# Sanoojan/VFace

Hardware: AMD Instinct MI355X
Metric: swapped frames/sec at 512x512, 50-step DDIM (higher is better)
Workload: dtype f16

## Files before the change

### include/vface_hip.h

```cpp
#ifndef VFACE_HIP_H
#define VFACE_HIP_H

#include <stddef.h>
#include <stdint.h>

#ifdef __cplusplus
extern "C" {
#endif

#define VFACE_ABI_VERSION 8

#define VFACE_OK 0
#define VFACE_ERR_ARG (-1)
#define VFACE_ERR_ALIGN (-2)
#define VFACE_ERR_SHAPE (-3)
#define VFACE_ERR_DTYPE (-4)
#define VFACE_ERR_LAUNCH (-5)
#define VFACE_ERR_WORKSPACE (-6)

#define VFACE_F16 0
#define VFACE_BF16 1

#define VFACE_EPI_GEGLU 1
#define VFACE_EPI_OUT_F32 2
#define VFACE_TUNE_VARIANT(v) ((v) << 8)
#define VFACE_CONV_PAD_TRAILING 0x40000
#define VFACE_TUNE_NO_PERSISTENT 0x10000
#define VFACE_TUNE_PERSISTENT 0x20000
#define VFACE_TUNE_NO_PATCH 0x80000
#define VFACE_TUNE_PATCH 0x100000
#define VFACE_TUNE_GN8 0x8000000
#define VFACE_TUNE_NO_Q8 0x4000000
#define VFACE_TUNE_PATCH_BN160 0x2000000
#define VFACE_TUNE_F32_TRANSPOSE 0x1000000
#define VFACE_TUNE_BIG_TILE 0x10000000
#define VFACE_TUNE_NO_BIG_TILE 0x20000000
#define VFACE_TUNE_BIG_W256 0x200000
#define VFACE_TUNE_BIG_W320 0x400000

#define VFACE_FUSION_NONE 0
#define VFACE_FUSION_REPLACE 1
#define VFACE_FUSION_LINEAR 2

int vface_abi_version(void);
const char* vface_error_string(int code);
int vface_gemm_variants_built(void);

typedef struct vface_stream32 {
    const float* residual32;
    int64_t ldr32;
    float* out32;
    int64_t ldo32;
    const float* in_scale_shift;
// ... 191 lines not shown
```

### vface_amd/csrc/conv.hip

```cpp
#include <type_traits>
#include "common.hpp"
#include "vface_kernels.hpp"

namespace {

constexpr int TP = 16;

template <class TT, int NT, int KH, int KW, bool DIAG = false, bool GNT = false, int RM = -1, bool Q8 = false>
__global__ __launch_bounds__(512, 2) void conv_patch_kernel(GemmParams p) {
    using E = typename TT::elem;
    using V8 = typename TT::v8;
    constexpr int BN = 32 * NT;
    constexpr int TAPS = KH * KW;
    static_assert(!Q8 || (KH == 3 && KW == 3 && NT == 4), "the 8x8 form: 3x3 windows, 128-channel tiles");
    constexpr int PW = Q8 ? 20 : TP + KW - 1, PH = Q8 ? 20 : TP + KH - 1, NPIX = PW * PH;
    constexpr int NPIECES = (NPIX + 7) / 8;
    constexpr int PATCH_BYTES = NPIECES * 1024;
    constexpr int PPW = (NPIECES + 7) / 8;
    constexpr int BPIECES = BN / 8;
    constexpr int BSLOT = BN * 128;
    constexpr int NB_HI = (BPIECES + 7) / 8, NB_LO = BPIECES / 8;
    constexpr int NB_SPLIT = BPIECES % 8;
    constexpr int NSLOT = (TAPS % 3 == 0) ? 3 : 4;
    static_assert(TAPS % NSLOT == 0 && (NSLOT - 1) * BSLOT < 65536, "slot offsets must fold into the ds_read immediate");
    extern __shared__ __attribute__((aligned(16))) unsigned char smem_raw[];
    unsigned char* sB = smem_raw;
    unsigned char* sP = smem_raw + NSLOT * BSLOT;
    constexpr bool GNF = GNT && KH == 3;
    unsigned char* sT = sP + 2 * PATCH_BYTES;
// ... 9 lines not shown
        if constexpr (!DIAG) return 0ull;
        unsigned long long tt;
        __builtin_amdgcn_sched_barrier(0);
        asm volatile("s_memtime %0\n\ts_waitcnt lgkmcnt(0)" : "=s"(tt)::"memory");
        __builtin_amdgcn_sched_barrier(0);
        return tt;
    };
    const unsigned long long d_t0 = stamp();
    const unsigned long long d_sync = 0, d_issue = 0, d_comp = 0;

    const int tiles_x = p.W / TP, tiles_y = p.H / TP, tiles_img = tiles_x * tiles_y;
    const int nimg_all = p.M / (p.OH * p.OW);
    const int ntm = Q8 ? (nimg_all + 3) / 4 : nimg_all * tiles_img, ntn = p.N / BN;
    int tm, tn, sk = 0;
    {
        const int nwg = ntm * ntn * (Q8 ? p.split_k : 1), id = blockIdx.x;
        const int q = nwg >> 3, r = nwg & 7, xcd = id & 7, loc = id >> 3;
        int L = (xcd < r ? xcd * (q + 1) : r * (q + 1) + (xcd - r) * q) + loc;
        if constexpr (Q8) { sk = L / (ntm * ntn); L -= sk * (ntm * ntn); }
        const int GN = p.tile_group > 0 ? p.tile_group : 8;
        const int g = L / (GN * ntm);
        const int rem = L - g * (GN * ntm);
        const int gw = min(GN, ntn - g * GN);
        tm = rem / gw;
        tn = g * GN + (rem - tm * gw);
    }
    const int img = Q8 ? tm * 4 : tm / tiles_img, trem = Q8 ? 0 : tm - img * tiles_img;
    const int ty0 = Q8 ? 0 : (trem / tiles_x) * TP, tx0 = Q8 ? 0 : (trem - (trem / tiles_x) * tiles_x) * TP;
    const int n0 = tn * BN;

    const __amdgpu_buffer_rsrc_t rA = __builtin_amdgcn_make_buffer_rsrc(const_cast<void*>(p.A), 0, (int)p.a_bytes, 0x00020000);
    const __amdgpu_buffer_rsrc_t rA2 = __builtin_amdgcn_make_buffer_rsrc(const_cast<void*>(p.A2 ? p.A2 : p.A), 0, (int)(p.A2 ? p.a2_bytes : 0u), 0x00020000);
    const __amdgpu_buffer_rsrc_t rW = __builtin_amdgcn_make_buffer_rsrc(const_cast<void*>(p.Wt), 0, (int)p.w_bytes, 0x00020000);
    const bool gn = GNF && p.gn_ab != nullptr;
    const __amdgpu_buffer_rsrc_t rT = __builtin_amdgcn_make_buffer_rsrc(const_cast<float*>(gn ? p.gn_ab : (const float*)p.Wt), 0, (int)(gn ? p.gn_ab_bytes : 0u), 0x00020000);

    constexpr bool TAIL = KH == 3;
    unsigned poff[PPW], poff2[TAIL ? 4 : 1];
    const unsigned pch = (unsigned)((lane & 7) ^ ((lane >> 3) & 7));
#pragma unroll
    for (int i = 0; i < PPW; ++i) {
        const int pp = (wave + 8 * i) * 8 + (lane >> 3);
        const int py = pp / PW, px = pp - py * PW;
        if constexpr (Q8) {
            const int qy = py / 10, qx = px / 10, iy = py - qy * 10 - 1, ix = px - qx * 10 - 1, im = img + qy * 2 + qx;
            const bool ok = pp < NPIX && (unsigned)iy < 8u && (unsigned)ix < 8u && im < nimg_all;
            poff[i] = ok ? (unsigned)(((((long)im * 8 + iy) * 8 + ix) * p.lda + pch * 8) * ES) : OOB;
            continue;
        }
        const int iy = ty0 - p.pad + py, ix = tx0 - p.pad_x + px;
        const bool ok = pp < NPIX && (unsigned)iy < (unsigned)p.H && (unsigned)ix < (unsigned)p.W;
        poff[i] = ok ? (unsigned)(((((long)img * p.H + iy) * p.W + ix) * p.lda + pch * 8) * ES) : OOB;
    }
#pragma unroll
    for (int i = 0; i < (TAIL ? 4 : 0); ++i) {
        const int pp = (wave + 8 * i) * 8 + (lane >> 3);
        const int ly = pp >> 4, lx = pp & 15;
        if constexpr (Q8) {
            const int im = img + (ly >> 3) * 2 + (lx >> 3);
            poff2[i] = (p.A2 && im < nimg_all) ? (unsigned)(((((long)im * 8 + (ly & 7)) * 8 + (lx & 7)) * p.lda2 + pch * 8) * ES) : OOB;
            continue;
        }
        poff2[i] = p.A2 ? (unsigned)(((((long)img * p.H + ty0 + ly) * p.W + tx0 + lx) * p.lda2 + pch * 8) * ES) : OOB;
    }
    unsigned boff[NB_HI];
#pragma unroll
    for (int i = 0; i < NB_HI; ++i) {
        const int piece = wave + 8 * i;
        const int row = piece * 8 + (lane >> 3);
        const unsigned ch = (unsigned)((lane & 7) ^ ((row >> 1) & 7));
        boff[i] = (piece < BPIECES && n0 + row < p.N) ? (unsigned)((((long)(n0 + row)) * p.ldw + ch * 8) * ES) : OOB;
    }

    const int nchunks_all = p.Cin >> 6;
    int c_begin = 0, nchunks = nchunks_all;
    if constexpr (Q8) {
        const long total = (long)nchunks_all * TAPS + ((TAIL && p.A2) ? ((p.K - p.K1) >> 6) : 0);
        int prev = 0;
        for (int k = 1; k <= p.split_k; ++k) {
            int b = k == p.split_k ? nchunks_all : (int)((k * total / p.split_k + TAPS / 2) / TAPS);
            b = min(max(b, prev + 1), nchunks_all - (p.split_k - k));
            if (k == sk) c_begin = b;
            if (k == sk + 1) { nchunks = b; break; }
            prev = b;
        }
    }
    const int kt0 = c_begin * TAPS;
    const int T1 = (nchunks - c_begin) * TAPS;
    const int ntail = (TAIL && p.A2 && (!Q8 || sk == p.split_k - 1)) ? ((p.K - p.K1) >> 6) : 0;
    const int T = T1 + ntail;

    auto issue_B = [&](int kt, int slot) {
        if (DIAG && (p.flags & 0x200000) && kt >= 2) return;
        unsigned char* dst = sB + slot * BSLOT;
        const unsigned koff = (unsigned)(kt0 + kt) * 64u * ES;
#pragma unroll
        for (int i = 0; i < NB_HI; ++i) {
            if (i < NB_LO || wave < NB_SPLIT) {
                const unsigned off = boff[i] != OOB ? boff[i] + koff : OOB;
                __builtin_amdgcn_raw_ptr_buffer_load_lds(rW, LDS_PTR(dst + (wave + 8 * i) * 1024), 16, off, 0, 0, 0);
            }
        }
    };
    auto issue_P = [&](int c, int i) {
        if (DIAG && (p.flags & 0x200000) && c >= 1) return;
        const int piece = wave + 8 * i;
        if (piece < NPIECES) {
            const unsigned off = poff[i] != OOB ? poff[i] + (unsigned)c * 64u * ES : OOB;
            __builtin_amdgcn_raw_ptr_buffer_load_lds(rA, LDS_PTR(sP + (c & 1) * PATCH_BYTES + piece * 1024), 16, off, 0, 0, 0);
        }
    };
    auto issue_P2 = [&](int u, int i) {
        const unsigned off = poff2[TAIL ? i : 0] != OOB ? poff2[TAIL ? i : 0] + (unsigned)u * 64u * ES : OOB;
        __builtin_amdgcn_raw_ptr_buffer_load_lds(rA2, LDS_PTR(sP + ((nchunks + u) & 1) * PATCH_BYTES + (wave + 8 * i) * 1024), 16, off, 0, 0, 0);
    };

    auto issue_T = [&](int c) {
        if (gn && wave == 7) {
            const unsigned off = lane < 32 ? (unsigned)((((long)img * p.ld_gn_ab + c * 64) * 2) * 4 + lane * 16) : OOB;
            __builtin_amdgcn_raw_ptr_buffer_load_lds(rT, LDS_PTR(sT + (c & 1) * 1024), 16, off, 0, 0, 0);
        }
    };
    auto transform_P = [&](int c, int i) {
        const int piece = wave + 8 * i;
        if (piece < NPIECES && poff[i] != OOB) {
            unsigned char* a = sP + (c & 1) * PATCH_BYTES + piece * 1024 + lane * 16;
            const V8 v = *reinterpret_cast<const V8*>(a);
            const float4* tb = reinterpret_cast<const float4*>(sT + (c & 1) * 1024 + pch * 64);
            const float4 t0 = tb[0], t1 = tb[1], t2 = tb[2], t3 = tb[3];
            const float aa[8] = {t0.x, t0.z, t1.x, t1.z, t2.x, t2.z, t3.x, t3.z};
            const float bb[8] = {t0.y, t0.w, t1.y, t1.w, t2.y, t2.w, t3.y, t3.w};
            V8 o;
#pragma unroll
            for (int e = 0; e < 8; ++e) {
                float f = to_f32(v[e]) * aa[e] + bb[e];
                if (p.gn_silu) f = silu_f(f);
                o[e] = from_f32<E>(f);
            }
            *reinterpret_cast<V8*>(a) = o;
        }
    };

    f4_t acc[NT][4];
#pragma unroll
    for (int j = 0; j < NT; ++j)
#pragma unroll
        for (int i = 0; i < 4; ++i) acc[j][i] = f4_t{0.f, 0.f, 0.f, 0.f};

    constexpr bool WADR1 = (NSLOT - 1) * BSLOT + (NT - 1) * 2048 + 64 < 65536;
    const int wrow = wn * (BN / 2) + fr;
    const unsigned wadr0 = (unsigned)(wrow * 128 + ((fq ^ ((wrow >> 1) & 7)) << 4));
    unsigned wadrs[WADR1 ? 1 : NT];
    if constexpr (!WADR1) {
#pragma unroll
        for (int j = 0; j < NT; ++j) wadrs[j] = wadr0 + j * 2048;
    }
    auto wadr = [&](int j) -> unsigned { if constexpr (WADR1) return wadr0 + j * 2048; else return wadrs[j]; };
    const int lane_pp = Q8 ? (wm * 4 + (wm >= 2 ? 2 : 0)) * PW + fr + (fr >= 8 ? 2 : 0) : wm * 4 * PW + fr;

    V8 afX[4], bfX[NT], afY[4], bfY[NT];
    unsigned padr[4];
    bool abl_reads = false;
    auto read_h0 = [&](unsigned pbase, int ppk, int pw, unsigned wbase) {
        if (DIAG && abl_reads) return;
#pragma unroll
        for (int i = 0; i < 4; ++i) {
            const int pp = lane_pp + ppk + i * pw;
            padr[i] = pbase + (unsigned)(pp * 128) + (unsigned)((fq ^ (pp & 7)) << 4);
        }
#pragma unroll
        for (int i = 0; i < 4; ++i) afX[i] = *reinterpret_cast<const V8*>(smem_raw + padr[i]);
#pragma unroll
        for (int j = 0; j < NT; ++j) bfX[j] = *reinterpret_cast<const V8*>(sB + wbase + wadr(j));
    };
    auto read_h1 = [&](unsigned wbase) {
        if (DIAG && abl_reads) return;
#pragma unroll
        for (int i = 0; i < 4; ++i) afY[i] = *reinterpret_cast<const V8*>(smem_raw + (padr[i] ^ 64u));
#pragma unroll
        for (int j = 0; j < NT; ++j) bfY[j] = *reinterpret_cast<const V8*>(sB + wbase + (wadr(j) ^ 64u));
    };
    auto mfma_X = [&]() {
// ... 31 lines not shown
    if (nchunks > c_begin) {
#pragma unroll
        for (int i = 0; i < PPW; ++i) issue_P(c_begin, i);
        issue_T(c_begin);
    } else if constexpr (TAIL) {
        if (ntail > 0) {
#pragma unroll
            for (int i = 0; i < 4; ++i) issue_P2(0, i);
        }
    }
    issue_B(0, 0);
    if (T > 1) issue_B(1, 1 % NSLOT);

    const unsigned long long d_t1 = stamp();
    int kt = 0;
    for (int c = c_begin; c < nchunks; ++c) {
        const unsigned pbase = (unsigned)(NSLOT * BSLOT + (c & 1) * PATCH_BYTES);
        const bool next_window = c + 1 < nchunks;
#pragma unroll
        for (int tap = 0; tap < TAPS; ++tap) {
            period_sync(kt + 1 < T);
            if (GNF && gn) {
                if (tap == 0 && c == c_begin) {
#pragma unroll
                    for (int i = 0; i < PPW; ++i) transform_P(c_begin, i);
                    asm volatile("s_waitcnt lgkmcnt(0)" ::: "memory");
                    __builtin_amdgcn_s_barrier();
                    asm volatile("" ::: "memory");
                }
                if (tap >= 1 && tap <= PPW && next_window) transform_P(c + 1, tap - 1);
            }
            read_h0(pbase, (tap / KW) * PW + (tap % KW), PW, (unsigned)((tap % NSLOT) * BSLOT));
            __builtin_amdgcn_sched_barrier(0);
            if (late && kt > 0) { mfma_Y(); __builtin_amdgcn_sched_barrier(0); }
#pragma unroll
            for (int i = 0; i < PPW; ++i) {
                if (i % TAPS == tap) {
                    if (next_window) issue_P(c + 1, i);
                    else if (TAIL && ntail > 0 && i < 4) issue_P2(0, i);
                }
            }
            if (GNF && tap == 0 && next_window) issue_T(c + 1);
            if (kt + 2 < T) issue_B(kt + 2, (tap + 2) % NSLOT);
            __builtin_amdgcn_sched_barrier(0);
            if (!late && kt > 0) { mfma_Y(); __builtin_amdgcn_sched_barrier(0); }
            read_h1((unsigned)((tap % NSLOT) * BSLOT));
            __builtin_amdgcn_sched_barrier(0);
            mfma_X();
            __builtin_amdgcn_sched_barrier(0);
            ++kt;
            if (DIAG && (p.flags & 0x800000)) abl_reads = true;
        }
    }
    for (int u = 0; u < ntail; ++u) {
        period_sync(kt + 1 < T);
        const unsigned wb = (unsigned)((kt % NSLOT) * BSLOT);
        read_h0((unsigned)(NSLOT * BSLOT + ((nchunks + u) & 1) * PATCH_BYTES), wm * 4 * TP + fr - lane_pp, TP, wb);
        __builtin_amdgcn_sched_barrier(0);
        if (late && kt > 0) { mfma_Y(); __builtin_amdgcn_sched_barrier(0); }
        if (u + 1 < ntail) {
#pragma unroll
            for (int i = 0; i < 4; ++i) issue_P2(u + 1, i);
        }
        if (kt + 2 < T) issue_B(kt + 2, (kt + 2) % NSLOT);
        __builtin_amdgcn_sched_barrier(0);
        if (!late && kt > 0) { mfma_Y(); __builtin_amdgcn_sched_barrier(0); }
        read_h1(wb);
        __builtin_amdgcn_sched_barrier(0);
        mfma_X();
        __builtin_amdgcn_sched_barrier(0);
        ++kt;
    }
    mfma_Y();
    const unsigned long long d_t2 = stamp();

    if constexpr (Q8) {
        float* part = p.workspace + (long)sk * p.M * p.N;
        const int im = img + (wm >= 2 ? 2 : 0) + (fr >> 3);
        if (im < nimg_all) {
#pragma unroll
            for (int i = 0; i < 4; ++i) {
                const long m = (long)im * 64 + ((wm * 4 + i) & 7) * 8 + (fr & 7);
#pragma unroll
                for (int j = 0; j < NT; ++j)
                    *reinterpret_cast<float4*>(part + m * p.N + n0 + wn * (BN / 2) + j * 16 + fq * 4) =
                        make_float4(acc[j][i][0], acc[j][i][1], acc[j][i][2], acc[j][i][3]);
            }
        }
        return;
    }
    __syncthreads();
// ... 210 lines not shown
    hipLaunchKernelGGL(kern, dim3(ntm * ntn), dim3(512), lds, stream, q);
    return hipGetLastError() == hipSuccess ? VF_OK : VF_ERR_LAUNCH;
}

template <class TT>
int launch_patch_dtype(const GemmParams& p, int bn, hipStream_t stream) {
    if (p.KH == 3 && p.KW == 3) return bn == 160 ? launch_patch<TT, 5, 3, 3>(p, stream) : launch_patch<TT, 4, 3, 3>(p, stream);
    if (p.KH == 2 && p.KW == 2) return bn == 160 ? launch_patch<TT, 5, 2, 2>(p, stream) : launch_patch<TT, 4, 2, 2>(p, stream);
    return VF_ERR_SHAPE;
}

template <class TT>
int launch_q8(const GemmParams& p, hipStream_t stream) {
    constexpr int NT = 4, BN = 128, NPIECES = 50;
    const size_t lds = 2 * (size_t)NPIECES * 1024 + 3 * (size_t)BN * 128 + 2048;
    auto kern = conv_patch_kernel<TT, NT, 3, 3, false, false, 0, true>;
    static VfOncePerDevice attr_set;
    if (!attr_set.set_lds(reinterpret_cast<const void*>(kern), (int)lds)) return VF_ERR_LAUNCH;
    const int nimg = p.M / 64, ntm = (nimg + 3) / 4, ntn = p.N / BN;
    hipLaunchKernelGGL(kern, dim3(ntm * ntn * p.split_k), dim3(512), lds, stream, p);
    return hipGetLastError() == hipSuccess ? VF_OK : VF_ERR_LAUNCH;
}

}

int vf_conv_q8_split(const GemmParams& p) {
    if (p.mode != 1 || p.stride != 1 || p.upsample || p.out_phase || (p.Cin & 63) || p.gn_ab) return 0;
    if (p.H != 8 || p.W != 8 || p.OH != 8 || p.OW != 8 || p.KH != 3 || p.KW != 3 || p.ntaps != 9 || p.pad != 1 || p.pad_x != 1) return 0;
    if ((p.flags & (GEMM_GEGLU | GEMM_OUT_F32 | GEMM_NARROW_EPILOGUE | GEMM_NO_PATCH | 0x4000 | (0xF << 8))) || (p.N % 128)) return 0;
    if (p.A2 && ((p.K - p.K1) & 63)) return 0;
    if (p.rows_per_sample != 64 && p.rowbias) return 0;
    const int nchunks = p.Cin >> 6;
    const long tiles24 = 12L * (p.N / 128);
    int s = (int)(256 / tiles24);
    if (s > 8) s = 8;
    if (s > nchunks / 2) s = nchunks / 2;
    return s < 1 ? 0 : s;
}

int vf_launch_conv_q8(const GemmParams& p, int dtype, hipStream_t stream) {
    if (dtype == VF_DTYPE_F16) return launch_q8<F16>(p, stream);
    if (dtype == VF_DTYPE_BF16) return launch_q8<BF16>(p, stream);
    return VF_ERR_DTYPE;
}

namespace {
}

int vf_conv_kernel_choice(const GemmParams& p, int* arg) {
    if (arg) *arg = 0;
    if (p.mode != 1 || ((p.flags >> 8) & 0xF) || (p.flags & GEMM_NO_PATCH)) return 0;
    const int bn = vf_conv_patch_tile(p);
// ... 67 lines not shown
```

### vface_amd/csrc/gemm.hip

```cpp
#include <type_traits>

#include "common.hpp"
#include "vface_kernels.hpp"

namespace {

constexpr int BM = 128, BK = 64;
enum { MODE_PLAIN = 0, MODE_CONV_FAST = 1, MODE_CONV_GENERIC = 2 };

template <class TT, int MODE, int NT, bool DB, bool PERSIST, int RM = -1>
__global__ __launch_bounds__(256, 2) void gemm_kernel(GemmParams p) {
    using E = typename TT::elem;
    using V8 = typename TT::v8;
    constexpr int BN = 32 * NT;
    constexpr int BROUNDS = BN / 32;
    constexpr int A_ELEMS = BM * BK, B_ELEMS = BN * BK, STAGE = A_ELEMS + B_ELEMS;
    extern __shared__ __attribute__((aligned(16))) unsigned char smem_raw[];
    E* smem = reinterpret_cast<E*>(smem_raw);

    const int t = threadIdx.x;
    const int lane = t & 63;
    const int wave = __builtin_amdgcn_readfirstlane(t >> 6);
    const int wm = wave >> 1, wn = wave & 1;
    unsigned long long dbg_t0 = 0, dbg_t1 = 0, dbg_t2 = 0, dbg_e0 = 0, dbg_ew = 0, dbg_er = 0, dbg_es = 0;
// ... 895 lines not shown
        const unsigned long nimg = (unsigned long)(p.M / (p.OH * p.OW));
        const unsigned long gb = ((nimg - 1) * (unsigned long)p.ld_gn_ab + p.Cin) * 8ul;
        if (gb >= 0xFFFFFFF0ul) return VF_ERR_SHAPE;
        p.gn_ab_bytes = (unsigned)gb;
    }
    if (vf_conv_in16_ok(p)) return vf_launch_conv_in16(p, dtype, stream);
    int karg = 0;
    const int kchoice = vf_conv_kernel_choice(p, &karg);
    if (kchoice == 1) return vf_launch_conv_patch(p, dtype, stream);
    if (kchoice == 2 && p.workspace) {
        const int s = karg;
        if (s && p.workspace_bytes >= (long)s * p.M * p.N * 4 && !((uintptr_t)p.workspace & 15) && (p.M % 64) == 0 &&
            !(p.residual && (((uintptr_t)p.residual & 15) || (p.ldr & 7))) && !(p.ldc & 7) && !((uintptr_t)p.C & 15)) {
            p.split_k = s;
            const int rc = vf_launch_conv_q8(p, dtype, stream);
            if (rc != VF_OK) return rc;
            if (dtype == VF_DTYPE_F16) hipLaunchKernelGGL(splitk_reduce_kernel<F16>, dim3((p.M + 63) / 64, (p.N + 255) / 256), dim3(256), 0, stream, p);
            else hipLaunchKernelGGL(splitk_reduce_kernel<BF16>, dim3((p.M + 63) / 64, (p.N + 255) / 256), dim3(256), 0, stream, p);
            return hipGetLastError() == hipSuccess ? VF_OK : VF_ERR_LAUNCH;
        }
    }
    if (p.mode == 0 && (p.flags & GEMM_PATCH) && !((p.flags >> 8) & 0xF) && vf_gemm_patch_tile(p)) return vf_launch_gemm_patch(p, dtype, stream);
    if (p.mode == 0 && vf_gemm_big_choice(p)) return vf_launch_gemm_big(p, dtype, stream);
    if (p.gn_ab) return VF_ERR_SHAPE;
    const int variant = pick_variant(p);
    if ((p.res_f32 || p.C32) && variant != 5 && variant != 6) return VF_ERR_SHAPE;
    if (p.mode == 1 && (p.ntaps != 9 || p.out_phase || p.A2) && variant != 5 && variant != 6) return VF_ERR_SHAPE;
    if (p.workspace && !p.out_phase && (variant == 5 || variant == 6) && !((p.flags >> 8) & 0xF) && !(p.flags & 0x4000)) {
        const int s = split_for(p.M, p.N, p.K, p.flags, p.rows_per_sample);
        if (s > 1 && p.workspace_bytes >= (long)s * p.M * p.N * 4 && !((uintptr_t)p.workspace & 15) &&
            !(p.residual && (((uintptr_t)p.residual & 15) || (p.ldr & 7))) && !(p.ldc & 7) && !((uintptr_t)p.C & 15)) {
// ... 15 lines not shown
```

### vface_amd/csrc/vface_kernels.hpp

```cpp
#pragma once
#include <hip/hip_runtime.h>
#include <stdint.h>

#include <atomic>

struct VfOncePerDevice {
    std::atomic<unsigned long long> done{0};
    bool set_lds(const void* kern, int bytes) {
        int dev = 0;
        if (hipGetDevice(&dev) != hipSuccess) return false;
        const unsigned long long bit = 1ull << (dev & 63);
        if (done.load(std::memory_order_acquire) & bit) return true;
        if (hipFuncSetAttribute(kern, hipFuncAttributeMaxDynamicSharedMemorySize, bytes) != hipSuccess) return false;
        done.fetch_or(bit, std::memory_order_release);
        return true;
    }
};

enum { GEMM_GEGLU = 1, GEMM_OUT_F32 = 2, GEMM_NO_XCD_REMAP = 0x1000, GEMM_NO_SETPRIO = 0x2000, GEMM_NARROW_EPILOGUE = 0x8000, GEMM_NO_PERSIST = 0x10000, GEMM_PERSIST = 0x20000,
       GEMM_NO_PATCH = 0x80000, GEMM_PATCH = 0x100000, GEMM_GN8 = 0x8000000 , GEMM_NO_Q8 = 0x4000000 , GEMM_PATCH_BN160 = 0x2000000 , GEMM_F32_TRANSPOSE = 0x1000000 ,
       GEMM_BIG = 0x10000000 , GEMM_NO_BIG = 0x20000000 ,
       GEMM_BIG_W256 = 0x200000 , GEMM_BIG_W320 = 0x400000  };

struct GemmParams {
    int mode;
    const void* A;
    long lda;
    const void* A2;
    long lda2;
    int K1, a2_row_mod;
    const void* Wt;
    long ldw;
    int Kw;
    int M, N, K;
    int H, W, Cin, OH, OW, stride, upsample;
    int pad;
// ... 28 lines not shown
};
long vf_splitk_workspace_bytes(int M, int N, int K, int flags, int rows_per_sample);
bool vf_gemm_variants_built();
int vf_launch_gemm(const GemmParams& p, int dtype, hipStream_t stream);
int vf_conv_patch_tile(const GemmParams& p);
int vf_conv_kernel_choice(const GemmParams& p, int* arg);
int vf_launch_conv_patch(const GemmParams& p, int dtype, hipStream_t stream);
int vf_gemm_patch_tile(const GemmParams& p);
int vf_launch_gemm_patch(const GemmParams& p, int dtype, hipStream_t stream);
bool vf_gemm_big_ok(const GemmParams& p);
bool vf_gemm_big_choice(const GemmParams& p);
int vf_launch_gemm_big(const GemmParams& p, int dtype, hipStream_t stream);
bool vf_conv_in16_ok(const GemmParams& p);
int vf_launch_conv_in16(const GemmParams& p, int dtype, hipStream_t stream);
int vf_conv_q8_split(const GemmParams& p);
int vf_launch_conv_q8(const GemmParams& p, int dtype, hipStream_t stream);
bool vf_attention_shared_scores_supported(int dh, int v_sets);

struct FfnParams {
    const float* x32; long ldx;
    const float* gamma; const float* beta; float eps;
    const void* W1;
    const float* b1;
    const void* W2p;
    const float* b2;
    void* out16; long ldo;
    float* out32; long ldo32;
    int M, C;
    const void* att; long ldatt;
    const float* resid; long ldr;
// ... 156 lines not shown
```

### vface_amd/hip.py

```python
from __future__ import annotations

import ctypes as C
import os
from typing import Optional, Tuple

import torch

_HERE = os.path.dirname(os.path.abspath(__file__))
LIB_PATH = os.environ.get("VFACE_HIP_LIB") or os.path.join(_HERE, "lib", "libvface_hip.so")

F16, BF16 = 0, 1
EPI_GEGLU, EPI_OUT_F32 = 1, 2
CONV_PAD_TRAILING = 0x40000
TUNE_NO_PATCH, TUNE_PATCH = 0x80000, 0x100000
TUNE_GN8 = 0x8000000
TUNE_NO_Q8 = 0x4000000
TUNE_PATCH_BN160 = 0x2000000
TUNE_F32_TRANSPOSE = 0x1000000
TUNE_NO_PERSISTENT, TUNE_PERSISTENT = 0x10000, 0x20000
TUNE_BIG_W256, TUNE_BIG_W320 = 0x200000, 0x400000
TUNE_BIG_TILE, TUNE_NO_BIG_TILE = 0x10000000, 0x20000000
FUSION_NONE, FUSION_REPLACE, FUSION_LINEAR = 0, 1, 2

_i64, _i32, _f32, _vp, _sz = C.c_int64, C.c_int, C.c_float, C.c_void_p, C.c_size_t


class Stream32(C.Structure):
    _fields_ = [("residual32", _vp), ("ldr32", _i64), ("out32", _vp), ("ldo32", _i64),
                ("in_scale_shift", _vp), ("ld_scale_shift", _i64), ("in_silu", _i32)]


_s32p = C.POINTER(Stream32)

SIGNATURES = {
    "vface_abi_version": (C.c_int, []),
    "vface_error_string": (C.c_char_p, [_i32]),
# ... 174 lines not shown
        return False


def splitk_workspace(device, M: int, N: int, K: int, flags: int = 0, rows_per_sample: int = 1):
    need = load().vface_splitk_workspace_bytes(M, N, K, flags, rows_per_sample)
    if need <= 0:
        return None, 0
    key = str(device) if _ws_domain == 0 else f"{device}#{_ws_domain}"
    ws = _splitk_ws.get(key)
    if ws is None or ws.numel() < need:
        ws = torch.empty(need, dtype=torch.uint8, device=device)
        _splitk_ws[key] = ws
    return ws, ws.numel()


def gemm(a: torch.Tensor, wt: torch.Tensor, out: torch.Tensor, *, M: int, N: int, K: int, lda: int, ldc: int,
         ldw: Optional[int] = None, bias=None, rowbias=None, rows_per_sample: int = 1, residual=None, ldr: int = 0,
         a2=None, lda2: int = 0, k1: int = 0, a2_row_mod: int = 0, flags: int = 0, colstats=None, split_k: bool = True,
         residual32=None, out32=None):
    lib = load()
    ws, ws_bytes = splitk_workspace(a.device, M, N, K, flags, rows_per_sample) if split_k else (None, 0)
    rc = lib.vface_gemm(_p(a), lda, _p(a2), lda2, k1, a2_row_mod, _p(wt), ldw if ldw is not None else K, M, N, K,
                        _p(bias), _p(rowbias), rows_per_sample, rowbias.stride(0) if rowbias is not None else 0,
                        _p(residual), ldr, _p(out), ldc, _p(zeros_page(a.device)), flags, dtype_code(a.dtype),
                        _p(colstats), colstats.stride(0) // 2 if colstats is not None else 0, _p(ws), ws_bytes, _stream(),
                        _s32(residual32, out32))
    _check(rc, "vface_gemm")


def conv3x3(x: torch.Tensor, wt: torch.Tensor, out: torch.Tensor, *, nimg: int, H: int, W: int, cin: int, cout: int,
            ldx: int, ldy: int, stride: int = 1, upsample: bool = False, bias=None, rowbias=None, residual=None,
            ldr: int = 0, flags: int = 0, colstats=None, split_k: bool = True, residual32=None, out32=None, gn_ab=None,
            gn_silu: bool = False):
    lib = load()
    vh, vw = (2 * H, 2 * W) if upsample else (H, W)
    M = nimg * ((vh - 1) // stride + 1) * ((vw - 1) // stride + 1)
    ws, ws_bytes = splitk_workspace(x.device, M, cout, 9 * cin, flags, M // nimg) if split_k else (None, 0)
    rc = lib.vface_conv3x3(_p(x), ldx, nimg, H, W, cin, _p(wt), 9 * cin, cout, stride, int(upsample), _p(bias),
                           _p(rowbias), rowbias.stride(0) if rowbias is not None else 0, _p(residual), ldr, _p(out),
                           ldy, _p(zeros_page(x.device)), flags, dtype_code(x.dtype), _p(colstats),
                           colstats.stride(0) // 2 if colstats is not None else 0, _p(ws), ws_bytes, _stream(),
                           _s32(residual32, out32, gn_ab, gn_silu))
    _check(rc, "vface_conv3x3")


def conv_uses_patch_kernel(H: int, W: int, cin: int, cout: int, window: int = 3, stride: int = 1, upsample: bool = False,
                           flags: int = 0) -> int:
    return int(load().vface_conv_uses_patch_kernel(H, W, cin, cout, window, stride, int(upsample), flags))

# ... 497 lines not shown
    lib = load()
    for py in (0, 1):
        for px in (0, 1):
            rc = lib.vface_upsample2x_conv3x3_phase(_p(x), ldx, nimg, H, W, cin, _p(wt_phases[2 * py + px]), 4 * cin, cout, py, px,
                                                    _p(bias), _p(rowbias), rowbias.stride(0) if rowbias is not None else 0,
                                                    _p(out), ldy, _p(zeros_page(x.device)), flags, dtype_code(x.dtype),
                                                    _p(colstats), colstats.stride(0) // 2 if colstats is not None else 0,
                                                    _stream(), _s32(None, out32))
            _check(rc, "vface_upsample2x_conv3x3_phase")


def conv3x3_plus_1x1(x: torch.Tensor, x2: torch.Tensor, wt: torch.Tensor, out: torch.Tensor, *, nimg: int, H: int, W: int,
                     cin: int, c2: int, cout: int, ldx: int, ldx2: int, ldy: int, bias=None, rowbias=None, flags: int = 0,
                     colstats=None, split_k: bool = True, out32=None, gn_ab=None, gn_silu: bool = False):
    lib = load()
    M, K = nimg * H * W, 9 * cin + c2
    ws, ws_bytes = splitk_workspace(x.device, M, cout, K, flags, H * W) if split_k else (None, 0)
    rc = lib.vface_conv3x3_plus_1x1(_p(x), ldx, nimg, H, W, cin, _p(x2), ldx2, c2, _p(wt), K, cout, _p(bias), _p(rowbias),
                                    rowbias.stride(0) if rowbias is not None else 0, _p(out), ldy, _p(zeros_page(x.device)),
                                    flags, dtype_code(x.dtype), _p(colstats),
                                    colstats.stride(0) // 2 if colstats is not None else 0, _p(ws), ws_bytes, _stream(),
                                    _s32(None, out32, gn_ab, gn_silu))
    _check(rc, "vface_conv3x3_plus_1x1")


CLIP_PATCH, CLIP_PATCH_K, CLIP_PATCH_KP = 14, 588, 640
ACT_QUICK_GELU, ACT_GELU_ERF = 0, 1


def clip_patches(img: torch.Tensor, out: torch.Tensor, *, B: int, grid: int, H: int, W: int, ldo: int, prep: bool, mask=None,
# ... 43 lines not shown
```

Before: 8.371.

## Fold Q8 conv split-K into one workgroup with fused epilogue

Adds a FOLD variant of the 8x8-image 3x3 conv kernel. When there are many output tiles and K is short, each workgroup runs every split-K share itself and sums the partial accumulators in registers, instead of launching split_k times as many workgroups that write fp32 partials to HBM. The kernel then does bias, rowbias, residual, output and column statistics in its own epilogue, so the separate reduce kernel is skipped. In exchange there are fewer workgroups (less parallelism), extra accumulator registers, and patch offsets recomputed on each load. Env var VFACE_SPLIT_IN_WG=0 or the new flags force the old path.

```diff
diff --git a/include/vface_hip.h b/include/vface_hip.h
--- a/include/vface_hip.h
+++ b/include/vface_hip.h
@@ -37,6 +37,8 @@
 #define VFACE_TUNE_NO_BIG_TILE 0x20000000
 #define VFACE_TUNE_BIG_W256 0x200000
 #define VFACE_TUNE_BIG_W320 0x400000
+#define VFACE_TUNE_SPLIT_HBM 0x10
+#define VFACE_TUNE_SPLIT_IN_WG 0x20
 
 #define VFACE_FUSION_NONE 0
 #define VFACE_FUSION_REPLACE 1
diff --git a/vface_amd/csrc/conv.hip b/vface_amd/csrc/conv.hip
--- a/vface_amd/csrc/conv.hip
+++ b/vface_amd/csrc/conv.hip
@@ -6,13 +6,14 @@
 
 constexpr int TP = 16;
 
-template <class TT, int NT, int KH, int KW, bool DIAG = false, bool GNT = false, int RM = -1, bool Q8 = false>
+template <class TT, int NT, int KH, int KW, bool DIAG = false, bool GNT = false, int RM = -1, bool Q8 = false, bool FOLD = false>
 __global__ __launch_bounds__(512, 2) void conv_patch_kernel(GemmParams p) {
     using E = typename TT::elem;
     using V8 = typename TT::v8;
     constexpr int BN = 32 * NT;
     constexpr int TAPS = KH * KW;
     static_assert(!Q8 || (KH == 3 && KW == 3 && NT == 4), "the 8x8 form: 3x3 windows, 128-channel tiles");
+    static_assert(!FOLD || (Q8 && !DIAG && !GNT), "the in-workgroup split exists for the 8x8 form only");
     constexpr int PW = Q8 ? 20 : TP + KW - 1, PH = Q8 ? 20 : TP + KH - 1, NPIX = PW * PH;
     constexpr int NPIECES = (NPIX + 7) / 8;
     constexpr int PATCH_BYTES = NPIECES * 1024;
@@ -52,10 +53,10 @@
     const int ntm = Q8 ? (nimg_all + 3) / 4 : nimg_all * tiles_img, ntn = p.N / BN;
     int tm, tn, sk = 0;
     {
-        const int nwg = ntm * ntn * (Q8 ? p.split_k : 1), id = blockIdx.x;
+        const int nwg = ntm * ntn * ((Q8 && !FOLD) ? p.split_k : 1), id = blockIdx.x;
         const int q = nwg >> 3, r = nwg & 7, xcd = id & 7, loc = id >> 3;
         int L = (xcd < r ? xcd * (q + 1) : r * (q + 1) + (xcd - r) * q) + loc;
-        if constexpr (Q8) { sk = L / (ntm * ntn); L -= sk * (ntm * ntn); }
+        if constexpr (Q8 && !FOLD) { sk = L / (ntm * ntn); L -= sk * (ntm * ntn); }
         const int GN = p.tile_group > 0 ? p.tile_group : 8;
         const int g = L / (GN * ntm);
         const int rem = L - g * (GN * ntm);
@@ -74,24 +75,27 @@
     const __amdgpu_buffer_rsrc_t rT = __builtin_amdgcn_make_buffer_rsrc(const_cast<float*>(gn ? p.gn_ab : (const float*)p.Wt), 0, (int)(gn ? p.gn_ab_bytes : 0u), 0x00020000);
 
     constexpr bool TAIL = KH == 3;
-    unsigned poff[PPW], poff2[TAIL ? 4 : 1];
+    unsigned poff[FOLD ? 1 : PPW], poff2[TAIL ? 4 : 1];
     const unsigned pch = (unsigned)((lane & 7) ^ ((lane >> 3) & 7));
-#pragma unroll
-    for (int i = 0; i < PPW; ++i) {
+    auto q8_poff = [&](int i, int ln) -> unsigned {
+        const int pp = (wave + 8 * i) * 8 + (ln >> 3);
+        const int py = pp / PW, px = pp - py * PW;
+        const int qy = py / 10, qx = px / 10, iy = py - qy * 10 - 1, ix = px - qx * 10 - 1, im = img + qy * 2 + qx;
+        const bool ok = pp < NPIX && (unsigned)iy < 8u && (unsigned)ix < 8u && im < nimg_all;
+        const unsigned ch = (unsigned)((ln & 7) ^ ((ln >> 3) & 7));
+        return ok ? (unsigned)(((((long)im * 8 + iy) * 8 + ix) * p.lda + ch * 8) * ES) : OOB;
+    };
+#pragma unroll
+    for (int i = 0; i < (FOLD ? 0 : PPW); ++i) {
+        if constexpr (Q8) { poff[i] = q8_poff(i, lane); continue; }
         const int pp = (wave + 8 * i) * 8 + (lane >> 3);
         const int py = pp / PW, px = pp - py * PW;
-        if constexpr (Q8) {
-            const int qy = py / 10, qx = px / 10, iy = py - qy * 10 - 1, ix = px - qx * 10 - 1, im = img + qy * 2 + qx;
-            const bool ok = pp < NPIX && (unsigned)iy < 8u && (unsigned)ix < 8u && im < nimg_all;
-            poff[i] = ok ? (unsigned)(((((long)im * 8 + iy) * 8 + ix) * p.lda + pch * 8) * ES) : OOB;
-            continue;
-        }
         const int iy = ty0 - p.pad + py, ix = tx0 - p.pad_x + px;
         const bool ok = pp < NPIX && (unsigned)iy < (unsigned)p.H && (unsigned)ix < (unsigned)p.W;
         poff[i] = ok ? (unsigned)(((((long)img * p.H + iy) * p.W + ix) * p.lda + pch * 8) * ES) : OOB;
     }
 #pragma unroll
-    for (int i = 0; i < (TAIL ? 4 : 0); ++i) {
+    for (int i = 0; i < ((TAIL && !FOLD) ? 4 : 0); ++i) {
         const int pp = (wave + 8 * i) * 8 + (lane >> 3);
         const int ly = pp >> 4, lx = pp & 15;
         if constexpr (Q8) {
@@ -102,30 +106,35 @@
         poff2[i] = p.A2 ? (unsigned)(((((long)img * p.H + ty0 + ly) * p.W + tx0 + lx) * p.lda2 + pch * 8) * ES) : OOB;
     }
     unsigned boff[NB_HI];
-#pragma unroll
-    for (int i = 0; i < NB_HI; ++i) {
+    auto w_off = [&](int i, int ln) -> unsigned {
         const int piece = wave + 8 * i;
-        const int row = piece * 8 + (lane >> 3);
-        const unsigned ch = (unsigned)((lane & 7) ^ ((row >> 1) & 7));
-        boff[i] = (piece < BPIECES && n0 + row < p.N) ? (unsigned)((((long)(n0 + row)) * p.ldw + ch * 8) * ES) : OOB;
-    }
+        const int row = piece * 8 + (ln >> 3);
+        const unsigned ch = (unsigned)((ln & 7) ^ ((row >> 1) & 7));
+        return (piece < BPIECES && n0 + row < p.N) ? (unsigned)((((long)(n0 + row)) * p.ldw + ch * 8) * ES) : OOB;
+    };
+#pragma unroll
+    for (int i = 0; i < NB_HI; ++i) boff[i] = (FOLD && i) ? 0u : w_off(i, lane);
 
     const int nchunks_all = p.Cin >> 6;
     int c_begin = 0, nchunks = nchunks_all;
-    if constexpr (Q8) {
-        const long total = (long)nchunks_all * TAPS + ((TAIL && p.A2) ? ((p.K - p.K1) >> 6) : 0);
+    const long q8_total = Q8 ? (long)nchunks_all * TAPS + ((TAIL && p.A2) ? ((p.K - p.K1) >> 6) : 0) : 0;
+    auto share_end = [&](int k, int prev) -> int {
+        const int b = k == p.split_k ? nchunks_all : (int)((k * q8_total / p.split_k + TAPS / 2) / TAPS);
+        return min(max(b, prev + 1), nchunks_all - (p.split_k - k));
+    };
+    if constexpr (Q8 && !FOLD) {
         int prev = 0;
         for (int k = 1; k <= p.split_k; ++k) {
-            int b = k == p.split_k ? nchunks_all : (int)((k * total / p.split_k + TAPS / 2) / TAPS);
-            b = min(max(b, prev + 1), nchunks_all - (p.split_k - k));
+            const int b = share_end(k, prev);
             if (k == sk) c_begin = b;
             if (k == sk + 1) { nchunks = b; break; }
             prev = b;
         }
     }
+    int fold_k = 1, fold_end = FOLD ? share_end(1, 0) : 0;
     const int kt0 = c_begin * TAPS;
     const int T1 = (nchunks - c_begin) * TAPS;
-    const int ntail = (TAIL && p.A2 && (!Q8 || sk == p.split_k - 1)) ? ((p.K - p.K1) >> 6) : 0;
+    const int ntail = (TAIL && p.A2 && (!Q8 || FOLD || sk == p.split_k - 1)) ? ((p.K - p.K1) >> 6) : 0;
     const int T = T1 + ntail;
 
     auto issue_B = [&](int kt, int slot) {
@@ -135,7 +144,10 @@
 #pragma unroll
         for (int i = 0; i < NB_HI; ++i) {
             if (i < NB_LO || wave < NB_SPLIT) {
-                const unsigned off = boff[i] != OOB ? boff[i] + koff : OOB;
+                unsigned bo;
+                if constexpr (FOLD) bo = boff[0] + (unsigned)(i * 64) * (unsigned)p.ldw * ES;
+                else bo = boff[i];
+                const unsigned off = bo != OOB ? bo + koff : OOB;
                 __builtin_amdgcn_raw_ptr_buffer_load_lds(rW, LDS_PTR(dst + (wave + 8 * i) * 1024), 16, off, 0, 0, 0);
             }
         }
@@ -144,12 +156,27 @@
         if (DIAG && (p.flags & 0x200000) && c >= 1) return;
         const int piece = wave + 8 * i;
         if (piece < NPIECES) {
-            const unsigned off = poff[i] != OOB ? poff[i] + (unsigned)c * 64u * ES : OOB;
+            unsigned po;
+            if constexpr (FOLD) { int lv = lane; asm volatile("" : "+v"(lv)); po = q8_poff(i, lv); }
+            else po = poff[i];
+            const unsigned off = po != OOB ? po + (unsigned)c * 64u * ES : OOB;
             __builtin_amdgcn_raw_ptr_buffer_load_lds(rA, LDS_PTR(sP + (c & 1) * PATCH_BYTES + piece * 1024), 16, off, 0, 0, 0);
         }
     };
+    auto p2off = [&](int i) -> unsigned {
+        if constexpr (!FOLD) return poff2[TAIL ? i : 0];
+        else {
+            int lv = lane;
+            asm volatile("" : "+v"(lv));
+            const int pp = (wave + 8 * i) * 8 + (lv >> 3), ly = pp >> 4, lx = pp & 15;
+            const int im = img + (ly >> 3) * 2 + (lx >> 3);
+            const unsigned ch = (unsigned)((lv & 7) ^ ((lv >> 3) & 7));
+            return (p.A2 && im < nimg_all) ? (unsigned)(((((long)im * 8 + (ly & 7)) * 8 + (lx & 7)) * p.lda2 + ch * 8) * ES) : OOB;
+        }
+    };
     auto issue_P2 = [&](int u, int i) {
-        const unsigned off = poff2[TAIL ? i : 0] != OOB ? poff2[TAIL ? i : 0] + (unsigned)u * 64u * ES : OOB;
+        const unsigned o2 = p2off(i);
+        const unsigned off = o2 != OOB ? o2 + (unsigned)u * 64u * ES : OOB;
         __builtin_amdgcn_raw_ptr_buffer_load_lds(rA2, LDS_PTR(sP + ((nchunks + u) & 1) * PATCH_BYTES + (wave + 8 * i) * 1024), 16, off, 0, 0, 0);
     };
 
@@ -161,7 +188,7 @@
     };
     auto transform_P = [&](int c, int i) {
         const int piece = wave + 8 * i;
-        if (piece < NPIECES && poff[i] != OOB) {
+        if (piece < NPIECES && poff[FOLD ? 0 : i] != OOB) {
             unsigned char* a = sP + (c & 1) * PATCH_BYTES + piece * 1024 + lane * 16;
             const V8 v = *reinterpret_cast<const V8*>(a);
             const float4* tb = reinterpret_cast<const float4*>(sT + (c & 1) * 1024 + pch * 64);
@@ -184,6 +211,25 @@
     for (int j = 0; j < NT; ++j)
 #pragma unroll
         for (int i = 0; i < 4; ++i) acc[j][i] = f4_t{0.f, 0.f, 0.f, 0.f};
+    f4_t fsum[FOLD ? NT : 1][4];
+    if constexpr (FOLD) {
+#pragma unroll
+        for (int j = 0; j < NT; ++j)
+#pragma unroll
+            for (int i = 0; i < 4; ++i) fsum[j][i] = f4_t{0.f, 0.f, 0.f, 0.f};
+    }
+    auto fold_share = [&]() {
+        if constexpr (FOLD) {
+#pragma unroll
+            for (int j = 0; j < NT; ++j)
+#pragma unroll
+                for (int i = 0; i < 4; ++i) {
+#pragma unroll
+                    for (int e = 0; e < 4; ++e) fsum[j][i][e] = fsum[j][i][e] + acc[j][i][e];
+                    acc[j][i] = f4_t{0.f, 0.f, 0.f, 0.f};
+                }
+        }
+    };
 
     constexpr bool WADR1 = (NSLOT - 1) * BSLOT + (NT - 1) * 2048 + 64 < 65536;
     const int wrow = wn * (BN / 2) + fr;
@@ -198,12 +244,13 @@
 
     V8 afX[4], bfX[NT], afY[4], bfY[NT];
     unsigned padr[4];
+    int lane_pp_v = lane_pp;
     bool abl_reads = false;
     auto read_h0 = [&](unsigned pbase, int ppk, int pw, unsigned wbase) {
         if (DIAG && abl_reads) return;
 #pragma unroll
         for (int i = 0; i < 4; ++i) {
-            const int pp = lane_pp + ppk + i * pw;
+            const int pp = lane_pp_v + ppk + i * pw;
             padr[i] = pbase + (unsigned)(pp * 128) + (unsigned)((fq ^ (pp & 7)) << 4);
         }
 #pragma unroll
@@ -265,9 +312,21 @@
 
     const unsigned long long d_t1 = stamp();
     int kt = 0;
+    bool pendY = false;
     for (int c = c_begin; c < nchunks; ++c) {
         const unsigned pbase = (unsigned)(NSLOT * BSLOT + (c & 1) * PATCH_BYTES);
         const bool next_window = c + 1 < nchunks;
+        if constexpr (FOLD) {
+            asm volatile("" : "+v"(lane_pp_v));
+            if (c == fold_end) {
+                mfma_Y();
+                __builtin_amdgcn_sched_barrier(0);
+                pendY = false;
+                fold_share();
+                ++fold_k;
+                fold_end = share_end(fold_k, fold_end);
+            }
+        }
 #pragma unroll
         for (int tap = 0; tap < TAPS; ++tap) {
             period_sync(kt + 1 < T);
@@ -283,7 +342,7 @@
             }
             read_h0(pbase, (tap / KW) * PW + (tap % KW), PW, (unsigned)((tap % NSLOT) * BSLOT));
             __builtin_amdgcn_sched_barrier(0);
-            if (late && kt > 0) { mfma_Y(); __builtin_amdgcn_sched_barrier(0); }
+            if (late && (FOLD ? pendY : kt > 0)) { mfma_Y(); __builtin_amdgcn_sched_barrier(0); }
 #pragma unroll
             for (int i = 0; i < PPW; ++i) {
                 if (i % TAPS == tap) {
@@ -294,12 +353,13 @@
             if (GNF && tap == 0 && next_window) issue_T(c + 1);
             if (kt + 2 < T) issue_B(kt + 2, (tap + 2) % NSLOT);
             __builtin_amdgcn_sched_barrier(0);
-            if (!late && kt > 0) { mfma_Y(); __builtin_amdgcn_sched_barrier(0); }
+            if (!late && (FOLD ? pendY : kt > 0)) { mfma_Y(); __builtin_amdgcn_sched_barrier(0); }
             read_h1((unsigned)((tap % NSLOT) * BSLOT));
             __builtin_amdgcn_sched_barrier(0);
             mfma_X();
             __builtin_amdgcn_sched_barrier(0);
             ++kt;
+            if constexpr (FOLD) pendY = true;
             if (DIAG && (p.flags & 0x800000)) abl_reads = true;
         }
     }
@@ -325,7 +385,99 @@
     mfma_Y();
     const unsigned long long d_t2 = stamp();
 
-    if constexpr (Q8) {
+    if constexpr (FOLD) {
+        fold_share();
+        constexpr int TLD = BN + 4;
+        static_assert(256 * TLD * 4 <= NSLOT * BSLOT + 2 * PATCH_BYTES, "the tile image lies inside the rings and patches");
+        float* timg = reinterpret_cast<float*>(smem_raw);
+        __syncthreads();
+        {
+            const int qd = (wm >= 2 ? 2 : 0) + (fr >> 3);
+#pragma unroll
+            for (int i = 0; i < 4; ++i) {
+                float* dst = timg + (qd * 64 + ((wm * 4 + i) & 7) * 8 + (fr & 7)) * TLD + wn * (BN / 2) + fq * 4;
+#pragma unroll
+                for (int j = 0; j < NT; ++j)
+                    *reinterpret_cast<float4*>(dst + j * 16) = make_float4(fsum[j][i][0], fsum[j][i][1], fsum[j][i][2], fsum[j][i][3]);
+            }
+        }
+        __syncthreads();
+        const int qd = t >> 7, rg = (t >> 4) & 7, c8 = t & 15;
+        const int im = img + qd;
+        const bool live = im < nimg_all;
+        const int n = n0 + c8 * 8;
+        const E* res = p.res_f32 ? nullptr : reinterpret_cast<const E*>(p.residual);
+        const float* res32 = p.res_f32 ? reinterpret_cast<const float*>(p.residual) : nullptr;
+        E* Cout = reinterpret_cast<E*>(p.C);
+        float s8[8], q8[8];
+#pragma unroll
+        for (int e = 0; e < 8; ++e) s8[e] = q8[e] = 0.f;
+        if (live) {
+            float b8[8], rb8[8];
+#pragma unroll
+            for (int e = 0; e < 8; ++e) b8[e] = p.bias ? p.bias[n + e] : 0.f;
+            if (p.rowbias) {
+                const float* rb = p.rowbias + (long)(((long)im * 64) / p.rows_per_sample) * p.ld_rowbias + n;
+#pragma unroll
+                for (int e = 0; e < 8; ++e) rb8[e] = rb[e];
+            }
+#pragma unroll
+            for (int it = 0; it < 8; ++it) {
+                const int row = rg + it * 8;
+                const long m = (long)im * 64 + row;
+                const float* src = timg + (qd * 64 + row) * TLD + c8 * 8;
+                const float4 x0 = *reinterpret_cast<const float4*>(src), x1 = *reinterpret_cast<const float4*>(src + 4);
+                float v[8] = {x0.x, x0.y, x0.z, x0.w, x1.x, x1.y, x1.z, x1.w};
+#pragma unroll
+                for (int e = 0; e < 8; ++e) v[e] += b8[e];
+                if (p.rowbias) {
+#pragma unroll
+                    for (int e = 0; e < 8; ++e) v[e] += rb8[e];
+                }
+                if (res) {
+                    const V8 r8 = *reinterpret_cast<const V8*>(res + m * p.ldr + n);
+#pragma unroll
+                    for (int e = 0; e < 8; ++e) v[e] += to_f32(r8[e]);
+                }
+                if (res32) {
+                    const float* rp = res32 + m * p.ldr + n;
+                    const float4 a = *reinterpret_cast<const float4*>(rp), b = *reinterpret_cast<const float4*>(rp + 4);
+                    v[0] += a.x; v[1] += a.y; v[2] += a.z; v[3] += a.w; v[4] += b.x; v[5] += b.y; v[6] += b.z; v[7] += b.w;
+                }
+                V8 o;
+#pragma unroll
+                for (int e = 0; e < 8; ++e) o[e] = from_f32<E>(v[e]);
+                if (Cout) *reinterpret_cast<V8*>(Cout + m * p.ldc + n) = o;
+                if (p.C32) {
+                    float* d32 = p.C32 + m * p.ldc32 + n;
+                    *reinterpret_cast<float4*>(d32) = make_float4(v[0], v[1], v[2], v[3]);
+                    *reinterpret_cast<float4*>(d32 + 4) = make_float4(v[4], v[5], v[6], v[7]);
+                }
+#pragma unroll
+                for (int e = 0; e < 8; ++e) { const float f = p.C32 ? v[e] : to_f32(o[e]); s8[e] += f; q8[e] = __builtin_fmaf(f, f, q8[e]); }
+            }
+        }
+        if (p.colstats) {
+            float* red = timg;
+            __syncthreads();
+            if (live) {
+#pragma unroll
+                for (int e = 0; e < 8; ++e) {
+                    red[(((qd * 8 + rg) * BN) + c8 * 8 + e) * 2] = s8[e];
+                    red[(((qd * 8 + rg) * BN) + c8 * 8 + e) * 2 + 1] = q8[e];
+                }
+            }
+            __syncthreads();
+            if (live) {
+                const int col = t & 127;
+                float ss = 0.f, qq = 0.f;
+#pragma unroll
+                for (int l = 0; l < 8; ++l) { ss += red[(((qd * 8 + l) * BN) + col) * 2]; qq += red[(((qd * 8 + l) * BN) + col) * 2 + 1]; }
+                *reinterpret_cast<float2*>(p.colstats + ((long)im * p.ld_colstats + n0 + col) * 2) = make_float2(ss, qq);
+            }
+        }
+        return;
+    } else if constexpr (Q8) {
         float* part = p.workspace + (long)sk * p.M * p.N;
         const int im = img + (wm >= 2 ? 2 : 0) + (fr >> 3);
         if (im < nimg_all) {
@@ -566,11 +718,12 @@
 int launch_q8(const GemmParams& p, hipStream_t stream) {
     constexpr int NT = 4, BN = 128, NPIECES = 50;
     const size_t lds = 2 * (size_t)NPIECES * 1024 + 3 * (size_t)BN * 128 + 2048;
-    auto kern = conv_patch_kernel<TT, NT, 3, 3, false, false, 0, true>;
-    static VfOncePerDevice attr_set;
-    if (!attr_set.set_lds(reinterpret_cast<const void*>(kern), (int)lds)) return VF_ERR_LAUNCH;
+    const bool fold = vf_conv_q8_in_wg(p);
+    auto kern = fold ? conv_patch_kernel<TT, NT, 3, 3, false, false, -1, true, true> : conv_patch_kernel<TT, NT, 3, 3, false, false, 0, true>;
+    static VfOncePerDevice attr_set[2];
+    if (!attr_set[fold].set_lds(reinterpret_cast<const void*>(kern), (int)lds)) return VF_ERR_LAUNCH;
     const int nimg = p.M / 64, ntm = (nimg + 3) / 4, ntn = p.N / BN;
-    hipLaunchKernelGGL(kern, dim3(ntm * ntn * p.split_k), dim3(512), lds, stream, p);
+    hipLaunchKernelGGL(kern, dim3(ntm * ntn * (fold ? 1 : p.split_k)), dim3(512), lds, stream, p);
     return hipGetLastError() == hipSuccess ? VF_OK : VF_ERR_LAUNCH;
 }
 
@@ -588,6 +741,14 @@
     if (s > 8) s = 8;
     if (s > nchunks / 2) s = nchunks / 2;
     return s < 1 ? 0 : s;
+}
+
+bool vf_conv_q8_in_wg(const GemmParams& p) {
+    if (p.flags & GEMM_SPLIT_HBM) return false;
+    if (p.flags & GEMM_SPLIT_IN_WG) return true;
+    const long tiles = (long)((p.M / 64 + 3) / 4) * (p.N / 128);
+    const int ktiles = (p.Cin >> 6) * 9 + (p.A2 ? ((p.K - p.K1) >> 6) : 0);
+    return tiles >= 160 && ktiles <= 240;
 }
 
 int vf_launch_conv_q8(const GemmParams& p, int dtype, hipStream_t stream) {
diff --git a/vface_amd/csrc/gemm.hip b/vface_amd/csrc/gemm.hip
--- a/vface_amd/csrc/gemm.hip
+++ b/vface_amd/csrc/gemm.hip
@@ -933,7 +933,7 @@
             !(p.residual && (((uintptr_t)p.residual & 15) || (p.ldr & 7))) && !(p.ldc & 7) && !((uintptr_t)p.C & 15)) {
             p.split_k = s;
             const int rc = vf_launch_conv_q8(p, dtype, stream);
-            if (rc != VF_OK) return rc;
+            if (rc != VF_OK || vf_conv_q8_in_wg(p)) return rc;
             if (dtype == VF_DTYPE_F16) hipLaunchKernelGGL(splitk_reduce_kernel<F16>, dim3((p.M + 63) / 64, (p.N + 255) / 256), dim3(256), 0, stream, p);
             else hipLaunchKernelGGL(splitk_reduce_kernel<BF16>, dim3((p.M + 63) / 64, (p.N + 255) / 256), dim3(256), 0, stream, p);
             return hipGetLastError() == hipSuccess ? VF_OK : VF_ERR_LAUNCH;
diff --git a/vface_amd/csrc/vface_kernels.hpp b/vface_amd/csrc/vface_kernels.hpp
--- a/vface_amd/csrc/vface_kernels.hpp
+++ b/vface_amd/csrc/vface_kernels.hpp
@@ -20,6 +20,7 @@
 enum { GEMM_GEGLU = 1, GEMM_OUT_F32 = 2, GEMM_NO_XCD_REMAP = 0x1000, GEMM_NO_SETPRIO = 0x2000, GEMM_NARROW_EPILOGUE = 0x8000, GEMM_NO_PERSIST = 0x10000, GEMM_PERSIST = 0x20000,
        GEMM_NO_PATCH = 0x80000, GEMM_PATCH = 0x100000, GEMM_GN8 = 0x8000000 , GEMM_NO_Q8 = 0x4000000 , GEMM_PATCH_BN160 = 0x2000000 , GEMM_F32_TRANSPOSE = 0x1000000 ,
        GEMM_BIG = 0x10000000 , GEMM_NO_BIG = 0x20000000 ,
+       GEMM_SPLIT_HBM = 0x10 , GEMM_SPLIT_IN_WG = 0x20 ,
        GEMM_BIG_W256 = 0x200000 , GEMM_BIG_W320 = 0x400000  };
 
 struct GemmParams {
@@ -78,6 +79,7 @@
 bool vf_conv_in16_ok(const GemmParams& p);
 int vf_launch_conv_in16(const GemmParams& p, int dtype, hipStream_t stream);
 int vf_conv_q8_split(const GemmParams& p);
+bool vf_conv_q8_in_wg(const GemmParams& p);
 int vf_launch_conv_q8(const GemmParams& p, int dtype, hipStream_t stream);
 bool vf_attention_shared_scores_supported(int dh, int v_sets);
 
diff --git a/vface_amd/hip.py b/vface_amd/hip.py
--- a/vface_amd/hip.py
+++ b/vface_amd/hip.py
@@ -20,6 +20,7 @@
 TUNE_NO_PERSISTENT, TUNE_PERSISTENT = 0x10000, 0x20000
 TUNE_BIG_W256, TUNE_BIG_W320 = 0x200000, 0x400000
 TUNE_BIG_TILE, TUNE_NO_BIG_TILE = 0x10000000, 0x20000000
+TUNE_SPLIT_HBM, TUNE_SPLIT_IN_WG = 0x10, 0x20
 FUSION_NONE, FUSION_REPLACE, FUSION_LINEAR = 0, 1, 2
 
 _i64, _i32, _f32, _vp, _sz = C.c_int64, C.c_int, C.c_float, C.c_void_p, C.c_size_t
@@ -224,6 +225,12 @@
     return ws, ws.numel()
 
 
+def _split_form(flags: int) -> int:
+    if not (flags & (TUNE_SPLIT_HBM | TUNE_SPLIT_IN_WG)) and os.environ.get("VFACE_SPLIT_IN_WG", "1") == "0":
+        return flags | TUNE_SPLIT_HBM
+    return flags
+
+
 def gemm(a: torch.Tensor, wt: torch.Tensor, out: torch.Tensor, *, M: int, N: int, K: int, lda: int, ldc: int,
          ldw: Optional[int] = None, bias=None, rowbias=None, rows_per_sample: int = 1, residual=None, ldr: int = 0,
          a2=None, lda2: int = 0, k1: int = 0, a2_row_mod: int = 0, flags: int = 0, colstats=None, split_k: bool = True,
@@ -243,6 +250,7 @@
             ldr: int = 0, flags: int = 0, colstats=None, split_k: bool = True, residual32=None, out32=None, gn_ab=None,
             gn_silu: bool = False):
     lib = load()
+    flags = _split_form(flags)
     vh, vw = (2 * H, 2 * W) if upsample else (H, W)
     M = nimg * ((vh - 1) // stride + 1) * ((vw - 1) // stride + 1)
     ws, ws_bytes = splitk_workspace(x.device, M, cout, 9 * cin, flags, M // nimg) if split_k else (None, 0)
@@ -770,6 +778,7 @@
                      cin: int, c2: int, cout: int, ldx: int, ldx2: int, ldy: int, bias=None, rowbias=None, flags: int = 0,
                      colstats=None, split_k: bool = True, out32=None, gn_ab=None, gn_silu: bool = False):
     lib = load()
+    flags = _split_form(flags)
     M, K = nimg * H * W, 9 * cin + c2
     ws, ws_bytes = splitk_workspace(x.device, M, cout, K, flags, H * W) if split_k else (None, 0)
     rc = lib.vface_conv3x3_plus_1x1(_p(x), ldx, nimg, H, W, cin, _p(x2), ldx2, c2, _p(wt), K, cout, _p(bias), _p(rowbias),
```

New measurement: 8.331. Within noise of the previous version (-0.5%).
